# RhushabhVaghela/Custom-NVComp-with-ZSTD

Hardware: AMD Instinct MI355X
Metric: compress GB/s + ratio, 1 GB @ level 3, 64 KB chunks; libzstd round-trip OK (higher is better)
Workload: dtype u8; 1 GPU; C3: 16384 x 64 KiB chunks (1.00 GiB), level 3, independent frames; chunk_bytes=65536, chunks_total=16384, chunks_rank0=16384, level=3, parallelism=dp1 (contiguous chunk shards, RCCL all-gather of sizes inside the step), gathered_frame_bytes=388747049

## Files before the change

custom-nvcomp-with-zstd_amd/csrc/zh_lz.hip:

```cpp
#include "zh_common.h"
#include "zh_hash.h"
#include "zh_litpack.h"

#include <algorithm>
#include <type_traits>
#include <vector>

#if defined(ZH_STAMPS) || defined(ZH_INS_CHECK)
__device__ u32 g_fixups;
extern "C" __global__ void zh_read_fixups(u32 *out) { *out = g_fixups; g_fixups = 0; }
extern "C" u32 zh_fixups_host() {
  u32 *d = nullptr, h = 0;
  if (hipMalloc(&d, 4) != hipSuccess) return ~0u;
  hipLaunchKernelGGL(zh_read_fixups, dim3(1), dim3(1), 0, 0, d);
  (void)hipMemcpy(&h, d, 4, hipMemcpyDeviceToHost);
  (void)hipFree(d);
  return h;
}
#endif
#ifdef ZH_TIMELINE
__device__ unsigned long long g_tl[16 * 8];
extern "C" __global__ void zh_read_timeline(unsigned long long *out) {
  for (u32 i = threadIdx.x; i < 16 * 8; i += blockDim.x) { out[i] = g_tl[i]; g_tl[i] = 0; }
}
extern "C" int zh_timeline_host(unsigned long long *out128) {
  unsigned long long *d = nullptr;
  if (hipMalloc(&d, 16 * 8 * 8) != hipSuccess) return 1;
  hipLaunchKernelGGL(zh_read_timeline, dim3(1), dim3(128), 0, 0, d);
  hipError_t e = hipMemcpy(out128, d, 16 * 8 * 8, hipMemcpyDeviceToHost);
  (void)hipFree(d);
  return e == hipSuccess ? 0 : 1;
}
#define TL_DECL u64 tl_[6] = {0, 0, 0, 0, 0, 0}; u64 tl_prev = __builtin_amdgcn_s_memtime()
#define TL_MARK(ph) do { u64 const _t = __builtin_amdgcn_s_memtime(); tl_[ph] += _t - tl_prev; tl_prev = _t; } while (0)
#define TL_STEP() (tl_[5]++)
#define TL_FLUSH(w, lane) do { if ((lane) == 0) for (u32 _i = 0; _i < 6; _i++) atomicAdd(&g_tl[(w) * 8 + _i], (unsigned long long)tl_[_i]); } while (0)
#else
#define TL_DECL do { } while (0)
#define TL_MARK(ph) do { } while (0)
#define TL_STEP() do { } while (0)
#define TL_FLUSH(w, lane) do { } while (0)
#endif
namespace {

constexpr u32 K1_THREADS = 1024;
constexpr u32 K1_REDO = ~0u;
constexpr u32 NROUND = ZH_WINDOW / 64;
constexpr u32 SEGP = 32;
constexpr u32 NSEG = ZH_WINDOW / SEGP;
constexpr u32 INS_TID = 896;
constexpr u64 ROUND_TAB = 0x6abfff8ull;
constexpr u32 NWW = INS_TID / 64;
constexpr u32 TILES = ZH_WINDOW / ZH_TILE;
constexpr u32 TPL = ZH_TILE / 64;
constexpr u32 NCR = TILES * TPL / 2;
static_assert(NSEG == 64, "one walk lane per segment");
static_assert(INS_TID == 896 && NROUND == 32, "round split: waves 1..13 take 2, 7 x 3, 4 x 2 and 1 rounds");
static_assert((ROUND_TAB & 3) == 0 && (ROUND_TAB >> (2 * (INS_TID / 64))) == 0, "no length rounds on wave 0 or the inserters");
constexpr u32 REC_WAVE = 1;
static_assert(ZH_WINDOW % ZH_TILE == 0 && ZH_TILE % 64 == 0 && TILES * TPL % 2 == 0, "tiles tile windows");

constexpr u32 HL_SIZE = 1u << ZH_HASH_LOG_LONG;
constexpr u32 HS_SIZE = 1u << ZH_HASH_LOG_SHORT;
constexpr u32 T_PAD = 8;
constexpr u32 OFF_IN = 0;
constexpr u32 OFF_TL = OFF_IN + ZH_BLOCK_MAX + 16;
constexpr u32 OFF_TS = OFF_TL + 2 * (HL_SIZE + T_PAD);
constexpr u32 OFF_CI = OFF_TS + 2 * (HS_SIZE + T_PAD);
constexpr u32 CI_WORDS = ZH_WINDOW + 8;
__device__ __forceinline__ u32 cidx(u32 i) { return i; }
constexpr u32 OFF_HM = OFF_CI + 2 * 4 * CI_WORDS;
constexpr u32 LM_BUFS = 3;
constexpr u32 LB_BUFS = 2;
constexpr u32 STEPS_EXTRA = 3;
constexpr u32 OFF_SEGM = OFF_HM + 2 * 8 * NROUND;
__device__ __forceinline__ u32 segm(u32 par) { return par * NSEG; }
constexpr u32 ML_CAP = ((ZH_WINDOW + ZH_MIN_MATCH_SHORT - 1) / ZH_MIN_MATCH_SHORT + 12 + 3) & ~3u;
constexpr u32 OFF_ML = OFF_SEGM + 4 * LM_BUFS * NSEG;
constexpr u32 XQ_CAP = 196;
constexpr u32 OFF_XQ = OFF_ML + 2 * 8 * ML_CAP;
constexpr u32 OFF_MISC = OFF_XQ + 2 * XQ_CAP * NWW;
constexpr u32 OFF_LB = OFF_MISC + 4 * 16;
constexpr u32 LB_WORDS = NSEG + 4;
constexpr u32 K1_LDS = OFF_LB + 4 * LB_WORDS * LB_BUFS;
constexpr u32 ML_LO = 11, ML_LEN = 22, ML_OFF = 29, ML_CUM = 45;
constexpr u32 MISC_WNM = 0;
constexpr u32 MISC_PF = 12;
constexpr u32 MISC_NM = 4;
constexpr u32 MISC_ANY = 13;
constexpr u32 MISC_SCAN = 2;
constexpr u32 MISC_XCH = 8;
constexpr u32 MISC_RESF = 14;
static_assert(K1_LDS <= 163840 - 256, "K1 LDS budget");
static_assert(OFF_TL % 16 == 0 && OFF_CI % 16 == 0 && OFF_HM % 16 == 0 && OFF_MISC % 4 == 0, "alignment");


__device__ __forceinline__ u32 ffbl_raw(u32 x) {
  u32 r;
  __asm__("v_ffbl_b32 %0, %1" : "=v"(r) : "v"(x));
  return r;
}

constexpr u32 K1_DYN = 16;
__device__ __forceinline__ u8 *k1_lds() { return (u8 *)(__attribute__((address_space(3))) u8 *)(uintptr_t)K1_DYN; }

__device__ __forceinline__ void k1_barrier() {
  __builtin_amdgcn_fence(__ATOMIC_RELEASE, "workgroup", "local");
  __builtin_amdgcn_s_barrier();
  __builtin_amdgcn_fence(__ATOMIC_ACQUIRE, "workgroup", "local");
}

__device__ __forceinline__ void ld64u(const u32 *in32, u32 p, u32 &lo, u32 &hi) {
  u32 const w = p >> 2, sh = p & 3;
  u32 const w0 = in32[w], w1 = in32[w + 1], w2 = in32[w + 2];
  lo = __builtin_amdgcn_alignbyte(w1, w0, sh);
  hi = __builtin_amdgcn_alignbyte(w2, w1, sh);
}
// ... 710 lines not shown
    const u32 *const lm = sgm + segm(j % LM_BUFS);
    const u32 *const lb = lbx + (j & 1u) * LB_WORDS;
    if (nr) {
      if constexpr (DW) lit_rounds(in32, lm, lb, lit_out, nlit, wsj, r0, nr, lane);
      else lit_rounds_pos((const u8 *)in32, lm, lb, lit_out, nlit, wsj, r0, nr, lane);
    }
    nlit += (u32)__builtin_amdgcn_readfirstlane(lb[NSEG]);
  }
};
template <class LJ>
__device__ __forceinline__ bool idle_inserter_loop(u32 *misc_, u32 n, u32 wstart, u32 kprobe, u32 e0p, LJ &lj, u32 lane, bool lazy) {
  u32 const nwin = (n - wstart + ZH_WINDOW - 1) / ZH_WINDOW;
  for (u32 k = 0; k < nwin + STEPS_EXTRA; k++) {
    if (probe_dead(misc_, k, kprobe)) return true;
    k1_barrier();
    u32 const wsb = wstart + k * ZH_WINDOW;
    if (probe_dead_tm(k, kprobe, e0p, lazy, min(wsb, n) - (wsb - ZH_WINDOW))) return true;
    lj.step(k, lane);
  }
  return false;
}
template <bool LONG, bool TWO, class LJ>
__device__ __forceinline__ bool inserter_loop(const u32 *in32, u16 *T, u8 *ci8, u32 *misc_, u32 n, u32 lim, u32 lane, u32 *dbg, u32 wstart,
                                              u32 pmin, u32 span_s, u32 span_e, u32 kskip0, u32 kprobe, u32 e0p, LJ &lj, bool lazy) {
  u32 creg[NCR];
  if (span_s < span_e) insert_span<LONG>(in32, T, span_s, span_e, lane);
  insert_window<LONG, true>(in32, T, wstart, lim, lane, creg, NoCheck{}, false, pmin);
  u32 cwe = lookahead<LONG>(in32, T, min(wstart + (u32)ZH_WINDOW, n), lim, lane);
  bool skipc = false;
#ifdef ZH_STAMPS
  u32 st_ins = 0;
#endif
  u32 const nwin = (n - wstart + ZH_WINDOW - 1) / ZH_WINDOW;
  TL_DECL;
  for (u32 k = 0; k < nwin + STEPS_EXTRA; k++) {
    if (probe_dead(misc_, k, kprobe)) return true;
    u32 const wsb = wstart + k * ZH_WINDOW;
    if (k < nwin) {
      for (u32 it = 0; it < (1u << 22) && (u32)__builtin_amdgcn_readfirstlane(__atomic_load_n(&misc_[MISC_PF], __ATOMIC_RELAXED)) < k; it++)
        __builtin_amdgcn_s_sleep(1);
      TL_MARK(3);
      if (skipc) dump_window<LONG, ZH_SKIP_TILES>(ci8 + (k & 1u) * 4 * CI_WORDS, lane, creg, cwe);
      else dump_window<LONG, TILES>(ci8 + (k & 1u) * 4 * CI_WORDS, lane, creg, cwe);
    }
    TL_MARK(4);
    k1_barrier();
    TL_MARK(0);
    TL_STEP();
    if (probe_dead_tm(k, kprobe, e0p, lazy, min(wsb, n) - (wsb - ZH_WINDOW))) return true;
#ifdef ZH_STAMPS
    u64 const ti0 = __builtin_amdgcn_s_memtime();
#endif
    u32 const nx = wsb + ZH_WINDOW;
    skipc = skip_window(misc_, k + 1, kskip0);
    if (k + 1 < nwin) {
      bool resumed = false;
      auto const on_check = [&](bool h) { return resumed = resume_exchange<LONG, TWO>(misc_, k + 1, h, lane); };
      if (nx + ZH_WINDOW <= lim) insert_window<LONG, false>(in32, T, nx, lim, lane, creg, on_check, skipc, 0u);
      else insert_window<LONG, true>(in32, T, nx, lim, lane, creg, on_check, skipc, 0u);
      if (resumed) skipc = false;
      cwe = lookahead<LONG>(in32, T, min(nx + ZH_WINDOW, n), lim, lane);
    }
#ifdef ZH_STAMPS
    st_ins += (u32)(__builtin_amdgcn_s_memtime() - ti0);
#endif
    TL_MARK(1);
    lj.step(k, lane);
    TL_MARK(2);
  }
  TL_FLUSH(LONG ? 14u : 15u, lane);
#ifdef ZH_STAMPS
  if (LONG && lane == 0) dbg[16] = st_ins;
#endif
  (void)dbg;
  return false;
}

}

#ifdef ZH_STAMPS
#define ZH_STAMP(acc)                                           \
  do {                                                          \
    u64 _t = __builtin_amdgcn_s_memtime();                      \
    acc += (u32)(_t - stamp_prev);                              \
    stamp_prev = _t;                                            \
  } while (0)
#else
#define ZH_STAMP(acc) do { } while (0)
#endif

struct Prefetch {
  uint4 v[4];
  bool ok;
};
__device__ __forceinline__ const u8 *staged_region(const ZhBlockDesc &d, u32 &n) {
  u32 const pre = d.pre_n;
  n = pre + d.n;
  const u8 *const g = (pre && d.pre + pre == d.src) ? d.pre : (pre ? nullptr : d.src);
  return (d.n && g && (((uintptr_t)g) & 15) == 0 && (pre & 15) == 0 && (n & 15) == 0) ? g : nullptr;
}
__device__ __forceinline__ void prefetch_block(const ZhBlockDesc *__restrict__ blocks, u32 b, u32 nblocks, u32 tid, Prefetch &pf) {
  pf.ok = false;
  if (b >= nblocks) return;
  ZhBlockDesc const d = blocks[b];
  u32 n;
  const u8 *const g = staged_region(d, n);
  if (!g) return;
  pf.ok = true;
#pragma unroll
  for (u32 k = 0; k < 4; k++) {
    u32 const i = tid + K1_THREADS * k;
    pf.v[k] = i < (n >> 4) ? ((const uint4 *)g)[i] : make_uint4(0, 0, 0, 0);
  }
}

constexpr u64 K1_WAVE_MAP = 0xFEDCBA9876543210ull;
__device__ __forceinline__ bool block_any(bool v, u32 *flag, u32 tid) {
  if (__ballot(v) && (tid & 63) == 0) atomicOr(flag, 1u);
  k1_barrier();
  bool const r = *flag != 0;
  k1_barrier();
  if (tid == 0) *flag = 0;
  k1_barrier();
  return r;
}

__device__ __forceinline__ u32 k1_tid(u32 w) {
  u32 lane;
  __asm__ volatile("v_mbcnt_lo_u32_b32 %0, -1, 0\n\tv_mbcnt_hi_u32_b32 %0, -1, %0" : "=v"(lane));
  return (u32)((K1_WAVE_MAP >> (4 * w)) & 15u) << 6 | lane;
}
// ... 47 lines not shown
#pragma unroll
    for (u32 k = 0; k < 6; k++) w[k] = in32[j0 + k];
#pragma unroll
    for (u32 k = 0; k < 5; k++) v[k] = __builtin_amdgcn_alignbyte(w[k + 1], w[k], sh);
    u32 const lo[4] = {v[0], __builtin_amdgcn_alignbyte(v[1], v[0], 3), __builtin_amdgcn_alignbyte(v[2], v[1], 2), __builtin_amdgcn_alignbyte(v[3], v[2], 1)};
    u32 const hi[4] = {v[1], __builtin_amdgcn_alignbyte(v[2], v[1], 3), __builtin_amdgcn_alignbyte(v[3], v[2], 2), __builtin_amdgcn_alignbyte(v[4], v[3], 1)};
    u32 t[4], e[4];
#pragma unroll
    for (u32 u = 0; u < 4; u++) {
      t[u] = hash_long_sum(lo[u], hi[u]);
      e[u] = *slot(t[u]);
    }
#pragma unroll
    for (u32 u = 0; u < 4; u++) c += (4u * g + u < nm && e[u] - key(t[u]) < p0 + 3u * u) ? 1u : 0u;
  }
  u32 const wsum = lane_value(wave_scan_incl(c), 63);
  if (lane == 0 && wsum) atomicAdd(&misc[MISC_SCAN], wsum);
  k1_barrier();
  u32 const total = (u32)__builtin_amdgcn_readfirstlane(__atomic_load_n(&misc[MISC_SCAN], __ATOMIC_RELAXED));
  return total >= max(span >> ZH_SCAN_SHIFT, (u32)ZH_SCAN_MIN);
}

template <u32 MODE, bool SET>
__device__ __forceinline__ u32 lz_block(const ZhBlockDesc *__restrict__ blocks, ZhWorkspace ws, u32 b, u32 nblocks, u32 *s_take, Prefetch &pf, u32 wv, bool redo) {
  u8 *const smem = k1_lds();
  u8 *in = smem + OFF_IN;
  u32 *in32 = (u32 *)in;
  u16 *TL = (u16 *)(smem + OFF_TL), *TS = (u16 *)(smem + OFF_TS);
  u32 *ci = (u32 *)(smem + OFF_CI);
  u8 *ci8 = smem + OFF_CI;
  u64 *hm = (u64 *)(smem + OFF_HM);
  u32 *misc = (u32 *)(smem + OFF_MISC);

  u32 tid;
  __asm__ volatile("v_mov_b32 %0, %1" : "=v"(tid) : "v"(k1_tid(wv)));
  u32 const lane = tid & 63;
  ZhBlockDesc const d = blocks[b];
  if (tid == 0 && !redo) *s_take = atomicAdd(ws.ctr, 1u);
  if (d.n == 0) {
    k1_barrier();
    u32 const next_b = *s_take;
    prefetch_block(blocks, next_b, nblocks, tid, pf);
    return next_b;
  }
  u32 const pre = d.pre_n;
  u32 const n = pre + d.n;
  u32 *meta = ws.meta(b);
#ifdef ZH_STAMPS
  u64 const rt0 = __builtin_amdgcn_s_memrealtime();
  u64 stamp_prev = __builtin_amdgcn_s_memtime();
  u64 const mt0 = stamp_prev;
  u32 st_stage = 0, st_A = 0, st_X = 0, st_E1 = 0, st_Bmax = 0, st_Imax = 0, st_Bw = 0, st_B = 0, st_J = 0, st_E = 0, st_E2 = 0, st_rounds = 0, st_J1 = 0, st_J2 = 0, st_J3 = 0;
#endif

  const u8 *src = d.src;
  bool same = true;
  u32 nst;
  if (!redo && pf.ok && staged_region(d, nst)) {
    u32 const nv = n >> 4, pv = pre >> 4;
    u32 const f4 = src[0] * 0x01010101u;
#pragma unroll
    for (u32 k = 0; k < 4; k++) {
      u32 const i = tid + K1_THREADS * k;
      uint4 const v = pf.v[k];
      if (i < nv) {
// ... 26 lines not shown
  }
  if (tid < 16) in[n + tid] = 0;
  const u16 *dtab = ws.dtab;
  u32 dtab_P = ws.dtab_P;
  if constexpr (SET) {
    if ((d.flags & ZH_F_DICT) && (d.flags & ZH_F_FIRST)) {
      const ZhDictSetEntry *const e = ws.set + ws.item_ent[d.item];
      dtab_P = e->dtab_P;
      dtab = dtab_P ? e->dtab : nullptr;
    }
  }
  bool const use_dt = dtab && (d.flags & ZH_F_DICT) && (d.flags & ZH_F_FIRST) && pre >= 2 * ZH_DTAB_MARGIN && d.n >= 16 &&
                      dtab_P >= pre;
  bool const par_hist = !use_dt && pre >= 2 * ZH_TILE && d.n >= 16;
  u32 const pmin = (use_dt || par_hist) ? pre & ~(ZH_TILE - 1) : 0u;
  u32 const wstart = (use_dt || par_hist) ? (pre & ~(ZH_WINDOW - 1)) : 0u;
  u32 const span_s = use_dt ? pre - ZH_DTAB_MARGIN : 0u, span_e = use_dt ? pmin : 0u;
  u32 const kskip0 = pre / ZH_WINDOW + 3 - wstart / ZH_WINDOW;
  u32 const lim = n > ZH_HASH_READ ? n - ZH_HASH_READ : 0;
  u32 const a0 = pre / ZH_WINDOW, nwl = (lim + ZH_WINDOW - 1) / ZH_WINDOW;
  u32 const e0p = pre - a0 * ZH_WINDOW;
  u32 const kprobe0 = a0 + ZH_PROBE_WINDOWS + 1 <= nwl && e0p <= ZH_PROBE_MAX_E0 ? a0 + ZH_PROBE_WINDOWS + 1 - wstart / ZH_WINDOW : ~0u;
  u32 next_b = 0;
  if (use_dt) {
    u32 const delta = dtab_P - pre;
    const u32 *dt32 = (const u32 *)dtab;
    auto clip = [&](u32 e) { return e > delta ? e - delta : 0u; };
    for (u32 i = tid; i < (HL_SIZE + HS_SIZE) / 2; i += K1_THREADS) {
      u32 const w = dt32[i];
      u32 const v = clip(w & 0xFFFFu) | (clip(w >> 16) << 16);
      u32 const j = i < HL_SIZE / 2 ? i : i + T_PAD / 2;
      ((u32 *)TL)[j] = v;
    }
    if (tid < T_PAD) ((u16 *)TL)[tid < T_PAD / 2 ? HL_SIZE + tid : HL_SIZE + T_PAD + HS_SIZE + (tid - T_PAD / 2)] = 0;
  } else {
    for (u32 i = tid; i < (HL_SIZE + HS_SIZE + 2 * T_PAD) / 2; i += K1_THREADS) ((u32 *)TL)[i] = 0;
  }
  if (tid == 0) {
    misc[MISC_PF] = 0;
#pragma unroll
    for (u32 i = 0; i < 4; i++) misc[MISC_XCH + i] = 0;
  }
  if (!redo) {
    bool const rle = !block_any(!same, &misc[MISC_ANY], tid) && d.n >= 2;
    next_b = *s_take;
    prefetch_block(blocks, next_b, nblocks, tid, pf);
    if (rle) {
      if (tid == 0) {
        u32 one;
        __asm__ volatile("v_mov_b32 %0, 1" : "=v"(one));
        meta[0] = one - 1u; meta[1] = one - 1u; meta[2] = one;
      }
      return next_b;
    }
  } else {
    next_b = *s_take;
    k1_barrier();
  }
  if (par_hist) {
    for (u32 round = 0;; round++) {
      bool ch = false;
      for (u32 p = tid; p < pmin; p += K1_THREADS) {
        u32 lo, hi;
        ld64u(in32, p, lo, hi);
        u32 const hl = hash_of<true>(lo, hi), hs = hash_of<false>(lo, hi);
        u16 const v = (u16)(p + 1);
        if (round == 0) {
          TL[hl] = v;
          TS[hs] = v;
        } else {
          if (TL[hl] < v) { TL[hl] = v; ch = true; }
          if (TS[hs] < v) { TS[hs] = v; ch = true; }
        }
      }
      if (round == 0) k1_barrier();
      else if (!block_any(ch, &misc[MISC_ANY], tid)) break;
    }
  }

  ZH_STAMP(st_stage);
  u32 const kprobe = redo ? ~0u : kprobe0;
  bool dead = false;
  if (tid >= INS_TID) {
    __builtin_amdgcn_s_setprio(2);
    bool const lw = tid < INS_TID + 64;
    LitJob<two_tables<MODE>()> lj{in32, (u32 *)(smem + OFF_SEGM), (u32 *)(smem + OFF_LB), ws.lits(b), wstart, n, pre,
              two_tables<MODE>() && !lw ? LIT_ROUNDS / 2 : 0u, two_tables<MODE>() ? LIT_ROUNDS / 2 : (lw ? LIT_ROUNDS : 0u), 0u};
    if (tid >= INS_TID + 64)
      dead = inserter_loop<false, two_tables<MODE>()>(in32, TS, ci8, misc, n, lim, lane, ws.dbg(b), wstart, pmin, span_s, span_e, kskip0, kprobe, e0p, lj,
                                                      MODE != 2);
    else if (two_tables<MODE>())
      dead = inserter_loop<true, true>(in32, TL, ci8, misc, n, lim, lane, ws.dbg(b), wstart, pmin, span_s, span_e, kskip0, kprobe, e0p, lj, MODE != 2);
    else
      dead = idle_inserter_loop(misc, n, wstart, kprobe, e0p, lj, lane, MODE != 2);
    __builtin_amdgcn_s_setprio(0);
    if (!dead) return next_b;
  } else {
  u64 *const seq_out = ws.seq(b);
  u32 nseq_tot = 0, nlit_tot = 0, e_in = pre;
  u32 const tid_ = tid;
  u32 const wave = tid >> 6;
  u32 r_lo = 0;
  for (u32 w = 0; w < wave; w++) r_lo += rounds_of_mode<MODE>(w);
  u32 const r_hi = r_lo + rounds_of_mode<MODE>(wave);
  u32 *const ci0 = ci;
  u32 *const sgm = (u32 *)(smem + OFF_SEGM);
  u32 *const lbx = (u32 *)(smem + OFF_LB);
  u16 *const xq = (u16 *)(smem + OFF_XQ) + XQ_CAP * wave;
  u32 const nwin = (n - wstart + ZH_WINDOW - 1) / ZH_WINDOW;
  u64 *const mlist = (u64 *)(smem + OFF_ML);
  u32 nwalk_tot = 0;
  TL_DECL;
  u32 m3 = 0;
  bool skp_prev = false;
  for (u32 k = 0; k < nwin + STEPS_EXTRA; k++, m3 = m3 + 1 == LM_BUFS ? 0u : m3 + 1) {
    if (probe_dead(misc, k, kprobe)) {
      dead = true;
      break;
    }
    u32 const wsb = wstart + k * ZH_WINDOW;
    u32 const we = min(wsb + ZH_WINDOW, n);
    u32 const kb = k & 1u;
    bool const have = k < nwin && we > pre;
    u32 const wsp = wsb - ZH_WINDOW, wep = min(wsp + ZH_WINDOW, n);
    bool const prev = k >= 1 && k <= nwin && wep > pre;
    u32 const wsq = wsb - 2 * ZH_WINDOW;
    bool const prev2 = k >= 2 && k - 2 < nwin && min(wsq + ZH_WINDOW, n) > pre;
    u32 tid;
    __asm__ volatile("v_mov_b32 %0, %1" : "=v"(tid) : "v"(tid_));
    u32 const lane = tid & 63;
    u32 *const ciK = ci0 + kb * CI_WORDS, *const ciP = ci0 + (kb ^ 1u) * CI_WORDS;
    u64 *const tmK = hm + kb * NROUND, *const tmP = hm + (kb ^ 1u) * NROUND;
    static_assert(LM_BUFS == 3 && LB_BUFS == 2, "literal buffer rotation");
    u32 *const lmP = sgm + segm(m3 == 0 ? 2u : m3 - 1u);
    u32 *const lmQ = sgm + segm(m3 == 0 ? 1u : m3 == 1 ? 2u : 0u);
    u32 *const lbxq = lbx + kb * LB_WORDS;
    u64 *const mlP = mlist + (kb ^ 1u) * ML_CAP, *const mlQ = mlist + kb * ML_CAP;
    k1_barrier();
    TL_MARK(0);
    TL_STEP();
    if (probe_dead_tm(k, kprobe, e0p, MODE != 2, wep - wsp)) {
      dead = true;
      break;
    }
    ZH_STAMP(st_A);
    constexpr u32 RS = 2 * ZH_SKIP_TILES;
    static_assert(RS < NWW && (RS & 1) == 0, "miss-skip rounds");
    bool const skipk = have && skip_window_eff(misc, k, kskip0);
    if (skipk && wave != 0) {
      if constexpr (MODE == 2) {
        if (wave <= RS / L1_S) span_lengths_l1(in32, ciK, tmK, xq, wave - 1, wave, wsb, n, lane);
      } else {
        if (wave <= RS) span_lengths<MODE, 1>(in32, ciK, tmK, xq, wave - 1, wave, wsb, we, n, lim, lane, wave == RS, 0u);
      }
      for (u32 r = RS + wave - 1; r < NROUND; r += NWW - 1) {
        ciK[cidx(64 * r + lane)] = 0;
        if (lane == 0) tmK[r] = 0;
      }
      ZH_STAMP(st_B);
    } else if (MODE == 2 && have && wave != 0) {
      if (r_lo < r_hi) span_lengths_l1(in32, ciK, tmK, xq, r_lo, r_hi, wsb, n, lane);
      ZH_STAMP(st_B);
    } else if (have && wave != 0) {
      u32 la1 = 0;
      if (wave == NWW - 1) {
// ... 104 lines not shown
        if (v) seq_out[nseq_tot + j] = (u64)cum | ((u64)len << 17) | ((u64)e << 24) | ((u64)off << 36);
        if (e) {
          for (u32 g = (ms - e) / SEGP; g <= (ms - 1) / SEGP; g++) {
            u32 const a = max(ms - e, SEGP * g) - SEGP * g, bnd = min(ms - SEGP * g, SEGP);
            atomicAnd(&lmQ[g], ~bit_range32(a, bnd));
          }
        }
      }
      u32 const lc = (u32)__popc(lmQ[lane]), lincl = wave_scan_incl(lc);
      lbxq[lane] = lincl - lc;
      if (lane == 63) lbxq[NSEG] = lincl;
      nlit_tot += lane_value(lincl, 63);
      nseq_tot += nm;
    }
    if (wave != 0) TL_MARK(2);
    TL_MARK(3);
    ZH_STAMP(st_X);
    ZH_STAMP(st_E);
    TL_MARK(4);
    skp_prev = skipk;
  }
  TL_FLUSH(wave, lane);
  if (!dead) {
    if (tid_ == 64u * REC_WAVE) { meta[0] = nseq_tot; meta[1] = nlit_tot; meta[2] = 0; }
#ifdef ZH_STAMPS
    if (tid == 0) {
      u32 *dbg = ws.dbg(b);
      dbg[23] = (u32)rt0; dbg[24] = (u32)__builtin_amdgcn_s_memrealtime();
      dbg[25] = __builtin_amdgcn_s_getreg((31 << 11) | 4);
      dbg[26] = __builtin_amdgcn_s_getreg((31 << 11) | 20);
      dbg[27] = (u32)(__builtin_amdgcn_s_memtime() - mt0);
      dbg[40] = st_Bmax; dbg[41] = st_Imax; dbg[55] = st_J1; dbg[56] = st_J2; dbg[57] = st_J3;
      dbg[0] = st_stage; dbg[1] = st_A; dbg[2] = st_B; dbg[3] = st_J; dbg[4] = st_E; dbg[5] = st_rounds; dbg[20] = st_E2; dbg[21] = st_X; dbg[22] = st_E1;
    }
    if ((tid & 63) == 0 && tid < INS_TID) {
      u32 const w = tid >> 6;
      ws.dbg(b)[w < 12 ? 28 + w : 53 + (w - 12)] = st_B;
    }
#endif
    return next_b;
  }
  }
  u32 *const hw = (u32 *)(smem + OFF_CI);
  if (repeat_scan(in32, (u32 *)TL, hw, misc, pre, n, tid)) return K1_REDO;
  ZH_STAMP(st_E1);
  u32 const wave = tid >> 6;
// ... 25 lines not shown
    u32 w[5];
#pragma unroll
    for (u32 k = 0; k < 5; k++) w[k] = src32[4 * i + k];
    uint4 v;
    v.x = __builtin_amdgcn_alignbyte(w[1], w[0], sh);
    v.y = __builtin_amdgcn_alignbyte(w[2], w[1], sh);
    v.z = __builtin_amdgcn_alignbyte(w[3], w[2], sh);
    v.w = __builtin_amdgcn_alignbyte(w[4], w[3], sh);
    ((uint4 *)lit_out)[i] = v;
  }
  if (tid == 0) { meta[0] = 0; meta[1] = d.n; meta[2] = 0; }
  return next_b;
}

template <u32 MODE, bool SET = false>
__device__ __forceinline__ void lz_blocks(const ZhBlockDesc *__restrict__ blocks, u32 nblocks, ZhWorkspace ws) {
  extern __shared__ __attribute__((aligned(16))) u8 smem_dyn[];
  u8 *const smem = k1_lds();
  if (threadIdx.x == 0 && (u32)(uintptr_t)smem_dyn != K1_DYN) __builtin_trap();
  __shared__ u32 s_take;
  if (threadIdx.x == 0) {
    s_take = atomicAdd(ws.ctr, 1u);
    ((u32 *)(smem + OFF_MISC))[MISC_ANY] = 0;
  }
  k1_barrier();
  u32 b = s_take;
  Prefetch pf;
  u32 const wv = (u32)__builtin_amdgcn_readfirstlane(threadIdx.x >> 6);
  prefetch_block(blocks, b, nblocks, k1_tid(wv), pf);
  bool redo = false;
  while (b < nblocks) {
    u32 const r = (u32)__builtin_amdgcn_readfirstlane(lz_block<MODE, SET>(blocks, ws, b, nblocks, &s_take, pf, wv, redo));
    k1_barrier();
    redo = r == K1_REDO;
    b = redo ? b : r;
  }
}
extern "C" __global__ __launch_bounds__(K1_THREADS) void zh_lz_kernel(const ZhBlockDesc *__restrict__ blocks, u32 nblocks, ZhWorkspace ws) {
  lz_blocks<0>(blocks, nblocks, ws);
}
extern "C" __global__ __launch_bounds__(K1_THREADS) void zh_lz_short_kernel(const ZhBlockDesc *__restrict__ blocks, u32 nblocks, ZhWorkspace ws) {
  lz_blocks<1>(blocks, nblocks, ws);
}
extern "C" __global__ __launch_bounds__(K1_THREADS) void zh_lz_greedy_kernel(const ZhBlockDesc *__restrict__ blocks, u32 nblocks, ZhWorkspace ws) {
  lz_blocks<2>(blocks, nblocks, ws);
}
extern "C" __global__ __launch_bounds__(K1_THREADS) void zh_lz_set_kernel(const ZhBlockDesc *__restrict__ blocks, u32 nblocks, ZhWorkspace ws) {
  lz_blocks<0, true>(blocks, nblocks, ws);
}
extern "C" __global__ __launch_bounds__(K1_THREADS) void zh_lz_short_set_kernel(const ZhBlockDesc *__restrict__ blocks, u32 nblocks, ZhWorkspace ws) {
  lz_blocks<1, true>(blocks, nblocks, ws);
}
extern "C" __global__ __launch_bounds__(K1_THREADS) void zh_lz_greedy_set_kernel(const ZhBlockDesc *__restrict__ blocks, u32 nblocks, ZhWorkspace ws) {
  lz_blocks<2, true>(blocks, nblocks, ws);
}
template <u32 MODE>
// ... 35 lines not shown

namespace zh {
hipError_t lz_init() {
  for (const void *f : {(const void *)zh_lz_kernel, (const void *)zh_lz_short_kernel, (const void *)zh_lz_greedy_kernel,
                        (const void *)zh_lz_ranged_kernel, (const void *)zh_lz_short_ranged_kernel, (const void *)zh_lz_greedy_ranged_kernel,
                        (const void *)zh_lz_set_kernel, (const void *)zh_lz_short_set_kernel, (const void *)zh_lz_greedy_set_kernel}) {
    hipError_t const e = hipFuncSetAttribute(f, hipFuncAttributeMaxDynamicSharedMemorySize, (int)K1_LDS);
    if (e != hipSuccess) return e;
  }
  return hipSuccess;
}
u32 lz_dict_tables_P(size_t cn) {
  u32 const P = (u32)std::min(cn, (size_t)65535);
  return P < 2 * ZH_DTAB_MARGIN ? 0u : P;
}
hipError_t lz_dict_tables_batch(const ZhDictBuildJob *d_jobs, u32 count, u32 *tmp32, hipStream_t stream) {
  if (!count) return hipSuccess;
  hipError_t e = hipMemsetAsync(tmp32, 0, (size_t)count * 4 * (HL_SIZE + HS_SIZE), stream);
  if (e != hipSuccess) return e;
  hipLaunchKernelGGL(zh_dict_hash_batch_kernel, dim3((65535 - ZH_DTAB_MARGIN + 255) / 256, count), dim3(256), 0, stream, d_jobs, tmp32);
  hipLaunchKernelGGL(zh_dict_pack_batch_kernel, dim3((HL_SIZE + HS_SIZE + 255) / 256, count), dim3(256), 0, stream, d_jobs, (const u32 *)tmp32);
  return hipGetLastError();
}
void lz_launch(const ZhBlockDesc *d_descs, u32 nblocks, ZhWorkspace ws, u32 mode, hipStream_t stream) {
  int dev = 0, cus = 0;
  if (stream) (void)hipStreamGetDevice(stream, &dev);
  else (void)hipGetDevice(&dev);
  if (hipDeviceGetAttribute(&cus, hipDeviceAttributeMultiprocessorCount, dev) != hipSuccess || cus <= 0) cus = 256;
  u32 const grid = std::min(nblocks, (u32)cus);
  auto *const k = ws.set ? (mode == 2 ? zh_lz_greedy_set_kernel : mode == 1 ? zh_lz_short_set_kernel : zh_lz_set_kernel)
                         : (mode == 2 ? zh_lz_greedy_kernel : mode == 1 ? zh_lz_short_kernel : zh_lz_kernel);
  hipLaunchKernelGGL(k, dim3(grid), dim3(K1_THREADS), K1_LDS, stream, d_descs, nblocks, ws);
}
void lz_launch_ranged(const ZhBlockDesc *d_descs, u32 nblocks, ZhWorkspace ws, ZhClassRanges *d_ranges, hipStream_t stream) {
  int dev = 0, cus = 0;
  if (stream) (void)hipStreamGetDevice(stream, &dev);
  else (void)hipGetDevice(&dev);
  if (hipDeviceGetAttribute(&cus, hipDeviceAttributeMultiprocessorCount, dev) != hipSuccess || cus <= 0) cus = 256;
  u32 const grid = std::min(nblocks, (u32)cus);
  for (auto *const k : {zh_lz_greedy_ranged_kernel, zh_lz_short_ranged_kernel, zh_lz_ranged_kernel})
    hipLaunchKernelGGL(k, dim3(grid), dim3(K1_THREADS), K1_LDS, stream, d_descs, d_ranges, ws);
}
}

extern "C" void zh_test_lz_sizes(u32 *seq_cap, u32 *lit_bytes) { *seq_cap = ZH_SEQ_CAP; *lit_bytes = ZH_LIT_BYTES; }
extern "C" int zh_test_lz(const u8 *d_in, u32 nitems, u32 stride, const u32 *h_sizes, int mode, u64 *h_recs, u8 *h_lits, u32 *h_meta) {
  if (!nitems) return 0;
  std::vector<ZhBlockDesc> descs(nitems);
  for (u32 i = 0; i < nitems; i++) {
    if (h_sizes[i] > ZH_BLOCK_MAX) return 2;
    ZhBlockDesc d{};
    d.src = d_in + (size_t)i * stride;
    d.n = h_sizes[i];
    d.frame_size = h_sizes[i];
    d.item = i;
    d.flags = ZH_F_FIRST | ZH_F_LAST | ZH_F_DIRECT;
    descs[i] = d;
  }
  ZhBlockDesc *dd = nullptr;
  u8 *base = nullptr;
  u32 *ctr = nullptr;
  int rc = 0;
  if (zh::lz_init() != hipSuccess || hipMalloc(&dd, sizeof(ZhBlockDesc) * nitems) != hipSuccess ||
      hipMalloc(&base, (size_t)ZH_WS_BLOCK_BYTES * nitems) != hipSuccess || hipMalloc(&ctr, 4) != hipSuccess) {
    rc = 1;
  } else {
    (void)hipMemcpy(dd, descs.data(), sizeof(ZhBlockDesc) * nitems, hipMemcpyHostToDevice);
    (void)hipMemset(ctr, 0, 4);
    ZhWorkspace ws{base, ctr, nullptr, 0u};
    zh::lz_launch(dd, nitems, ws, (u32)mode, nullptr);
    if (hipDeviceSynchronize() != hipSuccess) rc = 1;
    for (u32 i = 0; i < nitems && !rc; i++) {
      u8 *const b = base + (size_t)i * ZH_WS_BLOCK_BYTES;
      (void)hipMemcpy(h_recs + (size_t)i * ZH_SEQ_CAP, b, ZH_SEQ_BYTES, hipMemcpyDeviceToHost);
      (void)hipMemcpy(h_lits + (size_t)i * ZH_LIT_BYTES, b + ZH_SEQ_BYTES, ZH_LIT_BYTES, hipMemcpyDeviceToHost);
      (void)hipMemcpy(h_meta + 4 * i, b + ZH_SEQ_BYTES + ZH_LIT_BYTES, 16, hipMemcpyDeviceToHost);
    }
  }
  (void)hipFree(dd);
  (void)hipFree(base);
  (void)hipFree(ctr);
  return rc;
}
```

Before: 92.95 GB/s.

## Pre-insert next block's first window into hash tables during current block's drain

During the drain steps at the end of a block, the inserter waves load the next block's first window into a new LDS shadow buffer, clear their hash table, insert that window and dump its candidates. The next block then skips its own table clearing and first-window insertion, which overlaps block-boundary startup with the previous block's tail. The table zeroing also becomes 16-byte vector stores. In exchange this adds LDS use, restructures the inserter loop into body and tail variants, and adds cross-block state that must stay consistent on redo paths.

```diff
diff --git a/custom-nvcomp-with-zstd_amd/csrc/zh_k1_boundary.h b/custom-nvcomp-with-zstd_amd/csrc/zh_k1_boundary.h
--- /dev/null
+++ b/custom-nvcomp-with-zstd_amd/csrc/zh_k1_boundary.h
@@ -0,0 +1,65 @@
+#pragma once
+#include "zh_block_plan.h"
+
+#if defined(__HIPCC__)
+#define ZH_K1B_HD __host__ __device__ inline
+#else
+#define ZH_K1B_HD inline
+#endif
+
+namespace zh_k1 {
+
+constexpr u32 K1_THREADS = 1024;
+constexpr u32 NROUND = ZH_WINDOW / 64;
+constexpr u32 SEGP = 32;
+constexpr u32 NSEG = ZH_WINDOW / SEGP;
+constexpr u32 INS_TID = 896;
+constexpr u32 NWW = INS_TID / 64;
+
+constexpr u32 HL_SIZE = 1u << ZH_HASH_LOG_LONG;
+constexpr u32 HS_SIZE = 1u << ZH_HASH_LOG_SHORT;
+constexpr u32 T_PAD = 8;
+constexpr u32 OFF_IN = 0;
+constexpr u32 OFF_TL = OFF_IN + ZH_BLOCK_MAX + 16;
+constexpr u32 OFF_TS = OFF_TL + 2 * (HL_SIZE + T_PAD);
+constexpr u32 OFF_CI = OFF_TS + 2 * (HS_SIZE + T_PAD);
+constexpr u32 CI_WORDS = ZH_WINDOW + 8;
+constexpr u32 OFF_HM = OFF_CI + 2 * 4 * CI_WORDS;
+constexpr u32 LM_BUFS = 3;
+constexpr u32 LB_BUFS = 2;
+constexpr u32 OFF_SEGM = OFF_HM + 2 * 8 * NROUND;
+constexpr u32 ML_CAP = ((ZH_WINDOW + ZH_MIN_MATCH_SHORT - 1) / ZH_MIN_MATCH_SHORT + 12 + 3) & ~3u;
+constexpr u32 OFF_ML = OFF_SEGM + 4 * LM_BUFS * NSEG;
+constexpr u32 XQ_CAP = 196;
+constexpr u32 XQ_WAVES = NWW - 1;
+constexpr u32 OFF_XQ = OFF_ML + 2 * 8 * ML_CAP;
+constexpr u32 OFF_MISC = OFF_XQ + 2 * XQ_CAP * XQ_WAVES;
+constexpr u32 MISC_WORDS = 16;
+constexpr u32 OFF_LB = OFF_MISC + 4 * MISC_WORDS;
+constexpr u32 LB_WORDS = NSEG + 4;
+constexpr u32 SHADOW_BYTES = ZH_WINDOW + 16;
+constexpr u32 OFF_SHADOW = (OFF_LB + 4 * LB_WORDS * LB_BUFS + 15u) & ~15u;
+constexpr u32 K1_LDS = OFF_SHADOW + SHADOW_BYTES;
+constexpr u32 K1_LDS_BUDGET = 163840 - 256;
+static_assert(K1_LDS <= K1_LDS_BUDGET, "K1 LDS budget");
+static_assert(OFF_TL % 16 == 0 && OFF_TS % 16 == 0 && OFF_CI % 16 == 0 && OFF_HM % 16 == 0 && OFF_MISC % 4 == 0 && OFF_SHADOW % 16 == 0,
+              "alignment");
+
+ZH_K1B_HD const u8 *zh_k1_staged_region(const ZhBlockDesc &d, u32 &n) {
+  u32 const pre = d.pre_n;
+  n = pre + d.n;
+  const u8 *const g = (pre && d.pre + pre == d.src) ? d.pre : (pre ? nullptr : d.src);
+  return (d.n && g && (((uintptr_t)g) & 15) == 0 && (pre & 15) == 0 && (n & 15) == 0) ? g : nullptr;
+}
+
+constexpr u32 ZH_K1_PRE_MIN = ZH_WINDOW + 16;
+static_assert(ZH_K1_PRE_MIN >= SHADOW_BYTES && ZH_K1_PRE_MIN > ZH_WINDOW + 1 + ZH_HASH_READ, "the lookahead positions are below lim");
+
+ZH_K1B_HD u32 zh_k1_windows(u32 n, u32 wstart) { return (n - wstart + ZH_WINDOW - 1) / ZH_WINDOW; }
+
+ZH_K1B_HD bool zh_k1_preinsert(bool next_ok, u32 next_pre_n, u32 next_n, bool redo, u32 nwin) {
+  return next_ok && next_pre_n == 0 && next_n >= ZH_K1_PRE_MIN && !redo && nwin >= 3;
+}
+ZH_K1B_HD u32 zh_k1_predump_step(u32 nwin) { return nwin + (nwin & 1u) + 1u; }
+
+}
diff --git a/custom-nvcomp-with-zstd_amd/csrc/zh_lz.hip b/custom-nvcomp-with-zstd_amd/csrc/zh_lz.hip
--- a/custom-nvcomp-with-zstd_amd/csrc/zh_lz.hip
+++ b/custom-nvcomp-with-zstd_amd/csrc/zh_lz.hip
@@ -1,5 +1,6 @@
 #include "zh_common.h"
 #include "zh_hash.h"
+#include "zh_k1_boundary.h"
 #include "zh_litpack.h"
 
 #include <algorithm>
@@ -19,15 +20,16 @@
 }
 #endif
 #ifdef ZH_TIMELINE
-__device__ unsigned long long g_tl[16 * 8];
+constexpr unsigned ZH_TL_WORDS = 16 * 8 + 8;
+__device__ unsigned long long g_tl[ZH_TL_WORDS];
 extern "C" __global__ void zh_read_timeline(unsigned long long *out) {
-  for (u32 i = threadIdx.x; i < 16 * 8; i += blockDim.x) { out[i] = g_tl[i]; g_tl[i] = 0; }
-}
-extern "C" int zh_timeline_host(unsigned long long *out128) {
+  for (u32 i = threadIdx.x; i < ZH_TL_WORDS; i += blockDim.x) { out[i] = g_tl[i]; g_tl[i] = 0; }
+}
+extern "C" int zh_timeline_host(unsigned long long *out136) {
   unsigned long long *d = nullptr;
-  if (hipMalloc(&d, 16 * 8 * 8) != hipSuccess) return 1;
+  if (hipMalloc(&d, ZH_TL_WORDS * 8) != hipSuccess) return 1;
   hipLaunchKernelGGL(zh_read_timeline, dim3(1), dim3(128), 0, 0, d);
-  hipError_t e = hipMemcpy(out128, d, 16 * 8 * 8, hipMemcpyDeviceToHost);
+  hipError_t e = hipMemcpy(out136, d, ZH_TL_WORDS * 8, hipMemcpyDeviceToHost);
   (void)hipFree(d);
   return e == hipSuccess ? 0 : 1;
 }
@@ -35,7 +37,17 @@
 #define TL_MARK(ph) do { u64 const _t = __builtin_amdgcn_s_memtime(); tl_[ph] += _t - tl_prev; tl_prev = _t; } while (0)
 #define TL_STEP() (tl_[5]++)
 #define TL_FLUSH(w, lane) do { if ((lane) == 0) for (u32 _i = 0; _i < 6; _i++) atomicAdd(&g_tl[(w) * 8 + _i], (unsigned long long)tl_[_i]); } while (0)
+#define TB_PARAM , u64 &tb_prev
+#define TB_ARG , tb_prev
+#define TB_MARK(i, t) do { u64 const _t = __builtin_amdgcn_s_memtime(); if (tb_prev && (t) == 0) atomicAdd(&g_tl[128 + (i)], (unsigned long long)(_t - tb_prev)); tb_prev = _t; } while (0)
+#define TB_COUNT(t) do { if (tb_prev && (t) == 0) atomicAdd(&g_tl[133], 1ull); } while (0)
+#define TB_RESET() (tb_prev = 0)
 #else
+#define TB_PARAM
+#define TB_ARG
+#define TB_MARK(i, t) do { } while (0)
+#define TB_COUNT(t) do { } while (0)
+#define TB_RESET() do { } while (0)
 #define TL_DECL do { } while (0)
 #define TL_MARK(ph) do { } while (0)
 #define TL_STEP() do { } while (0)
@@ -43,14 +55,9 @@
 #endif
 namespace {
 
-constexpr u32 K1_THREADS = 1024;
+using namespace zh_k1;
 constexpr u32 K1_REDO = ~0u;
-constexpr u32 NROUND = ZH_WINDOW / 64;
-constexpr u32 SEGP = 32;
-constexpr u32 NSEG = ZH_WINDOW / SEGP;
-constexpr u32 INS_TID = 896;
 constexpr u64 ROUND_TAB = 0x6abfff8ull;
-constexpr u32 NWW = INS_TID / 64;
 constexpr u32 TILES = ZH_WINDOW / ZH_TILE;
 constexpr u32 TPL = ZH_TILE / 64;
 constexpr u32 NCR = TILES * TPL / 2;
@@ -60,29 +67,9 @@
 constexpr u32 REC_WAVE = 1;
 static_assert(ZH_WINDOW % ZH_TILE == 0 && ZH_TILE % 64 == 0 && TILES * TPL % 2 == 0, "tiles tile windows");
 
-constexpr u32 HL_SIZE = 1u << ZH_HASH_LOG_LONG;
-constexpr u32 HS_SIZE = 1u << ZH_HASH_LOG_SHORT;
-constexpr u32 T_PAD = 8;
-constexpr u32 OFF_IN = 0;
-constexpr u32 OFF_TL = OFF_IN + ZH_BLOCK_MAX + 16;
-constexpr u32 OFF_TS = OFF_TL + 2 * (HL_SIZE + T_PAD);
-constexpr u32 OFF_CI = OFF_TS + 2 * (HS_SIZE + T_PAD);
-constexpr u32 CI_WORDS = ZH_WINDOW + 8;
 __device__ __forceinline__ u32 cidx(u32 i) { return i; }
-constexpr u32 OFF_HM = OFF_CI + 2 * 4 * CI_WORDS;
-constexpr u32 LM_BUFS = 3;
-constexpr u32 LB_BUFS = 2;
 constexpr u32 STEPS_EXTRA = 3;
-constexpr u32 OFF_SEGM = OFF_HM + 2 * 8 * NROUND;
 __device__ __forceinline__ u32 segm(u32 par) { return par * NSEG; }
-constexpr u32 ML_CAP = ((ZH_WINDOW + ZH_MIN_MATCH_SHORT - 1) / ZH_MIN_MATCH_SHORT + 12 + 3) & ~3u;
-constexpr u32 OFF_ML = OFF_SEGM + 4 * LM_BUFS * NSEG;
-constexpr u32 XQ_CAP = 196;
-constexpr u32 OFF_XQ = OFF_ML + 2 * 8 * ML_CAP;
-constexpr u32 OFF_MISC = OFF_XQ + 2 * XQ_CAP * NWW;
-constexpr u32 OFF_LB = OFF_MISC + 4 * 16;
-constexpr u32 LB_WORDS = NSEG + 4;
-constexpr u32 K1_LDS = OFF_LB + 4 * LB_WORDS * LB_BUFS;
 constexpr u32 ML_LO = 11, ML_LEN = 22, ML_OFF = 29, ML_CUM = 45;
 constexpr u32 MISC_WNM = 0;
 constexpr u32 MISC_PF = 12;
@@ -91,8 +78,9 @@
 constexpr u32 MISC_SCAN = 2;
 constexpr u32 MISC_XCH = 8;
 constexpr u32 MISC_RESF = 14;
+constexpr u32 MISC_PRE = 3;
 static_assert(K1_LDS <= 163840 - 256, "K1 LDS budget");
-static_assert(OFF_TL % 16 == 0 && OFF_CI % 16 == 0 && OFF_HM % 16 == 0 && OFF_MISC % 4 == 0, "alignment");
+static_assert(STEPS_EXTRA == 3 && MISC_PRE < MISC_WORDS && MISC_RESF + 1 < MISC_WORDS, "the drain has a step for the next block's dump");
 
 
 __device__ __forceinline__ u32 ffbl_raw(u32 x) {
@@ -849,26 +837,49 @@
 }
 template <bool LONG, bool TWO, class LJ>
 __device__ __forceinline__ bool inserter_loop(const u32 *in32, u16 *T, u8 *ci8, u32 *misc_, u32 n, u32 lim, u32 lane, u32 *dbg, u32 wstart,
-                                              u32 pmin, u32 span_s, u32 span_e, u32 kskip0, u32 kprobe, u32 e0p, LJ &lj, bool lazy) {
+                                              u32 pmin, u32 span_s, u32 span_e, u32 kskip0, u32 kprobe, u32 e0p, LJ &lj, bool lazy,
+                                              bool pre_done, u32 nxn, u32 nxb, const ZhBlockDesc *__restrict__ blocks) {
   u32 creg[NCR];
-  if (span_s < span_e) insert_span<LONG>(in32, T, span_s, span_e, lane);
-  insert_window<LONG, true>(in32, T, wstart, lim, lane, creg, NoCheck{}, false, pmin);
-  u32 cwe = lookahead<LONG>(in32, T, min(wstart + (u32)ZH_WINDOW, n), lim, lane);
+  u32 cwe = 0;
+  if (!pre_done) {
+    if (span_s < span_e) insert_span<LONG>(in32, T, span_s, span_e, lane);
+    insert_window<LONG, true>(in32, T, wstart, lim, lane, creg, NoCheck{}, false, pmin);
+    cwe = lookahead<LONG>(in32, T, min(wstart + (u32)ZH_WINDOW, n), lim, lane);
+  }
   bool skipc = false;
 #ifdef ZH_STAMPS
   u32 st_ins = 0;
 #endif
-  u32 const nwin = (n - wstart + ZH_WINDOW - 1) / ZH_WINDOW;
+  u32 const nwin = zh_k1_windows(n, wstart);
+  u32 const kdump = nxn ? zh_k1_predump_step(nwin) : ~0u;
   TL_DECL;
-  for (u32 k = 0; k < nwin + STEPS_EXTRA; k++) {
+  auto step = [&](u32 k, auto tail_c) __attribute__((always_inline)) -> bool {
+    constexpr bool TAIL = decltype(tail_c)::value;
     if (probe_dead(misc_, k, kprobe)) return true;
     u32 const wsb = wstart + k * ZH_WINDOW;
-    if (k < nwin) {
+    constexpr u32 SHV = SHADOW_BYTES / 16 - 1;
+    static_assert(SHV == 128, "two rows of 64 vectors and one more");
+    bool const fill = TAIL && nxn != 0 && k + 1 == nwin;
+    uint4 sv0 = make_uint4(0, 0, 0, 0), sv1 = sv0, sv2 = sv0;
+    if (fill) {
+      const uint4 *const g = (const uint4 *)blocks[nxb].src;
+      if (!TWO || LONG) { sv0 = g[lane]; sv2 = g[SHV]; }
+      if (!TWO || !LONG) sv1 = g[64 + lane];
+    }
+    if (TAIL && k == kdump) {
+      TL_MARK(3);
+      dump_window<LONG, TILES>(ci8, lane, creg, cwe);
+    } else if ((!TAIL || k < nwin) && !(pre_done && k == 0)) {
       for (u32 it = 0; it < (1u << 22) && (u32)__builtin_amdgcn_readfirstlane(__atomic_load_n(&misc_[MISC_PF], __ATOMIC_RELAXED)) < k; it++)
         __builtin_amdgcn_s_sleep(1);
       TL_MARK(3);
       if (skipc) dump_window<LONG, ZH_SKIP_TILES>(ci8 + (k & 1u) * 4 * CI_WORDS, lane, creg, cwe);
       else dump_window<LONG, TILES>(ci8 + (k & 1u) * 4 * CI_WORDS, lane, creg, cwe);
+    }
+    if (fill) {
+      uint4 *const sh = (uint4 *)(k1_lds() + OFF_SHADOW);
+      if (!TWO || LONG) { sh[lane] = sv0; if (lane == 0) sh[SHV] = sv2; }
+      if (!TWO || !LONG) sh[64 + lane] = sv1;
     }
     TL_MARK(4);
     k1_barrier();
@@ -878,9 +889,9 @@
 #ifdef ZH_STAMPS
     u64 const ti0 = __builtin_amdgcn_s_memtime();
 #endif
-    u32 const nx = wsb + ZH_WINDOW;
-    skipc = skip_window(misc_, k + 1, kskip0);
-    if (k + 1 < nwin) {
+    if constexpr (!TAIL) {
+      u32 const nx = wsb + ZH_WINDOW;
+      skipc = skip_window(misc_, k + 1, kskip0);
       bool resumed = false;
       auto const on_check = [&](bool h) { return resumed = resume_exchange<LONG, TWO>(misc_, k + 1, h, lane); };
       if (nx + ZH_WINDOW <= lim) insert_window<LONG, false>(in32, T, nx, lim, lane, creg, on_check, skipc, 0u);
@@ -894,7 +905,25 @@
     TL_MARK(1);
     lj.step(k, lane);
     TL_MARK(2);
-  }
+    if (TAIL && nxn != 0 && k + 1 == nwin) {
+      u32 zero;
+      __asm__ volatile("v_mov_b32 %0, 0" : "=v"(zero));
+      constexpr u32 TV = 2 * ((LONG ? HL_SIZE : HS_SIZE) + T_PAD) / 16;
+      static_assert(2 * (HL_SIZE + T_PAD) % 16 == 0 && 2 * (HS_SIZE + T_PAD) % 16 == 0, "a table is whole 16-B vectors");
+      for (u32 i = lane; i < TV; i += 64) ((uint4 *)T)[i] = make_uint4(zero, zero, zero, zero);
+      const u32 *const sh32 = (const u32 *)(k1_lds() + OFF_SHADOW);
+      u32 const nlim = nxn - (u32)ZH_HASH_READ;
+      insert_window<LONG, true>(sh32, T, 0u, nlim, lane, creg, NoCheck{}, false, 0u);
+      cwe = lookahead<LONG>(sh32, T, min((u32)ZH_WINDOW, nxn), nlim, lane);
+      if (!LONG && lane == 0) misc_[MISC_PRE] = nxb + 1u;
+      TL_MARK(1);
+    }
+    return false;
+  };
+  for (u32 k = 0; k + 1 < nwin; k++)
+    if (step(k, std::false_type{})) return true;
+  for (u32 k = nwin - 1; k < nwin + STEPS_EXTRA; k++)
+    if (step(k, std::true_type{})) return true;
   TL_FLUSH(LONG ? 14u : 15u, lane);
 #ifdef ZH_STAMPS
   if (LONG && lane == 0) dbg[16] = st_ins;
@@ -919,21 +948,20 @@
 struct Prefetch {
   uint4 v[4];
   bool ok;
+  u32 bn, bpre;
 };
-__device__ __forceinline__ const u8 *staged_region(const ZhBlockDesc &d, u32 &n) {
-  u32 const pre = d.pre_n;
-  n = pre + d.n;
-  const u8 *const g = (pre && d.pre + pre == d.src) ? d.pre : (pre ? nullptr : d.src);
-  return (d.n && g && (((uintptr_t)g) & 15) == 0 && (pre & 15) == 0 && (n & 15) == 0) ? g : nullptr;
-}
+__device__ __forceinline__ const u8 *staged_region(const ZhBlockDesc &d, u32 &n) { return zh_k1_staged_region(d, n); }
 __device__ __forceinline__ void prefetch_block(const ZhBlockDesc *__restrict__ blocks, u32 b, u32 nblocks, u32 tid, Prefetch &pf) {
   pf.ok = false;
+  pf.bn = pf.bpre = 0;
   if (b >= nblocks) return;
   ZhBlockDesc const d = blocks[b];
   u32 n;
   const u8 *const g = staged_region(d, n);
   if (!g) return;
   pf.ok = true;
+  pf.bn = d.n;
+  pf.bpre = d.pre_n;
 #pragma unroll
   for (u32 k = 0; k < 4; k++) {
     u32 const i = tid + K1_THREADS * k;
@@ -1027,7 +1055,7 @@
 }
 
 template <u32 MODE, bool SET>
-__device__ __forceinline__ u32 lz_block(const ZhBlockDesc *__restrict__ blocks, ZhWorkspace ws, u32 b, u32 nblocks, u32 *s_take, Prefetch &pf, u32 wv, bool redo) {
+__device__ __forceinline__ u32 lz_block(const ZhBlockDesc *__restrict__ blocks, ZhWorkspace ws, u32 b, u32 nblocks, u32 *s_take, Prefetch &pf, u32 wv, bool redo TB_PARAM) {
   u8 *const smem = k1_lds();
   u8 *in = smem + OFF_IN;
   u32 *in32 = (u32 *)in;
@@ -1046,6 +1074,7 @@
     k1_barrier();
     u32 const next_b = *s_take;
     prefetch_block(blocks, next_b, nblocks, tid, pf);
+    TB_RESET();
     return next_b;
   }
   u32 const pre = d.pre_n;
@@ -1118,6 +1147,8 @@
   u32 const e0p = pre - a0 * ZH_WINDOW;
   u32 const kprobe0 = a0 + ZH_PROBE_WINDOWS + 1 <= nwl && e0p <= ZH_PROBE_MAX_E0 ? a0 + ZH_PROBE_WINDOWS + 1 - wstart / ZH_WINDOW : ~0u;
   u32 next_b = 0;
+  bool const pre_done = !redo && (u32)__builtin_amdgcn_readfirstlane(misc[MISC_PRE]) == b + 1u;
+  u32 nxn = 0;
   if (use_dt) {
     u32 const delta = dtab_P - pre;
     const u32 *dt32 = (const u32 *)dtab;
@@ -1129,8 +1160,11 @@
       ((u32 *)TL)[j] = v;
     }
     if (tid < T_PAD) ((u16 *)TL)[tid < T_PAD / 2 ? HL_SIZE + tid : HL_SIZE + T_PAD + HS_SIZE + (tid - T_PAD / 2)] = 0;
-  } else {
-    for (u32 i = tid; i < (HL_SIZE + HS_SIZE + 2 * T_PAD) / 2; i += K1_THREADS) ((u32 *)TL)[i] = 0;
+  } else if (!pre_done) {
+    u32 zero;
+    __asm__ volatile("v_mov_b32 %0, 0" : "=v"(zero));
+    static_assert((HL_SIZE + HS_SIZE + 2 * T_PAD) % 8 == 0, "the tables are whole 16-B vectors");
+    for (u32 i = tid; i < (HL_SIZE + HS_SIZE + 2 * T_PAD) / 8; i += K1_THREADS) ((uint4 *)TL)[i] = make_uint4(zero, zero, zero, zero);
   }
   if (tid == 0) {
     misc[MISC_PF] = 0;
@@ -1141,12 +1175,16 @@
     bool const rle = !block_any(!same, &misc[MISC_ANY], tid) && d.n >= 2;
     next_b = *s_take;
     prefetch_block(blocks, next_b, nblocks, tid, pf);
+    u32 const nn = (u32)__builtin_amdgcn_readfirstlane(pf.bn), npre = (u32)__builtin_amdgcn_readfirstlane(pf.bpre);
+    bool const nok = (u32)__builtin_amdgcn_readfirstlane(pf.ok ? 1u : 0u) != 0;
+    nxn = zh_k1_preinsert(nok, npre, nn, redo, zh_k1_windows(n, wstart)) ? nn : 0u;
     if (rle) {
       if (tid == 0) {
         u32 one;
         __asm__ volatile("v_mov_b32 %0, 1" : "=v"(one));
         meta[0] = one - 1u; meta[1] = one - 1u; meta[2] = one;
       }
+      TB_RESET();
       return next_b;
     }
   } else {
@@ -1175,6 +1213,7 @@
   }
 
   ZH_STAMP(st_stage);
+  TB_MARK(2, tid);
   u32 const kprobe = redo ? ~0u : kprobe0;
   bool dead = false;
   if (tid >= INS_TID) {
@@ -1182,11 +1221,13 @@
     bool const lw = tid < INS_TID + 64;
     LitJob<two_tables<MODE>()> lj{in32, (u32 *)(smem + OFF_SEGM), (u32 *)(smem + OFF_LB), ws.lits(b), wstart, n, pre,
               two_tables<MODE>() && !lw ? LIT_ROUNDS / 2 : 0u, two_tables<MODE>() ? LIT_ROUNDS / 2 : (lw ? LIT_ROUNDS : 0u), 0u};
+    u32 const nxb = (u32)__builtin_amdgcn_readfirstlane(next_b);
     if (tid >= INS_TID + 64)
       dead = inserter_loop<false, two_tables<MODE>()>(in32, TS, ci8, misc, n, lim, lane, ws.dbg(b), wstart, pmin, span_s, span_e, kskip0, kprobe, e0p, lj,
-                                                      MODE != 2);
+                                                      MODE != 2, pre_done, nxn, nxb, blocks);
     else if (two_tables<MODE>())
-      dead = inserter_loop<true, true>(in32, TL, ci8, misc, n, lim, lane, ws.dbg(b), wstart, pmin, span_s, span_e, kskip0, kprobe, e0p, lj, MODE != 2);
+      dead = inserter_loop<true, true>(in32, TL, ci8, misc, n, lim, lane, ws.dbg(b), wstart, pmin, span_s, span_e, kskip0, kprobe, e0p, lj, MODE != 2,
+                                       pre_done, nxn, nxb, blocks);
     else
       dead = idle_inserter_loop(misc, n, wstart, kprobe, e0p, lj, lane, MODE != 2);
     __builtin_amdgcn_s_setprio(0);
@@ -1202,8 +1243,8 @@
   u32 *const ci0 = ci;
   u32 *const sgm = (u32 *)(smem + OFF_SEGM);
   u32 *const lbx = (u32 *)(smem + OFF_LB);
-  u16 *const xq = (u16 *)(smem + OFF_XQ) + XQ_CAP * wave;
-  u32 const nwin = (n - wstart + ZH_WINDOW - 1) / ZH_WINDOW;
+  u16 *const xq = (u16 *)(smem + OFF_XQ) + XQ_CAP * (wave ? wave - 1u : 0u);
+  u32 const nwin = zh_k1_windows(n, wstart);
   u64 *const mlist = (u64 *)(smem + OFF_ML);
   u32 nwalk_tot = 0;
   TL_DECL;
@@ -1212,6 +1253,7 @@
   for (u32 k = 0; k < nwin + STEPS_EXTRA; k++, m3 = m3 + 1 == LM_BUFS ? 0u : m3 + 1) {
     if (probe_dead(misc, k, kprobe)) {
       dead = true;
+      TB_RESET();
       break;
     }
     u32 const wsb = wstart + k * ZH_WINDOW;
@@ -1235,8 +1277,11 @@
     k1_barrier();
     TL_MARK(0);
     TL_STEP();
+    if (k == 0) TB_MARK(3, tid_);
+    if (k == nwin) TB_MARK(4, tid_);
     if (probe_dead_tm(k, kprobe, e0p, MODE != 2, wep - wsp)) {
       dead = true;
+      TB_RESET();
       break;
     }
     ZH_STAMP(st_A);
@@ -1387,6 +1432,8 @@
   }
   TL_FLUSH(wave, lane);
   if (!dead) {
+    TB_COUNT(tid_);
+    TB_MARK(0, tid_);
     if (tid_ == 64u * REC_WAVE) { meta[0] = nseq_tot; meta[1] = nlit_tot; meta[2] = 0; }
 #ifdef ZH_STAMPS
     if (tid == 0) {
@@ -1458,6 +1505,7 @@
   if (threadIdx.x == 0) {
     s_take = atomicAdd(ws.ctr, 1u);
     ((u32 *)(smem + OFF_MISC))[MISC_ANY] = 0;
+    ((u32 *)(smem + OFF_MISC))[MISC_PRE] = 0;
   }
   k1_barrier();
   u32 b = s_take;
@@ -1465,9 +1513,13 @@
   u32 const wv = (u32)__builtin_amdgcn_readfirstlane(threadIdx.x >> 6);
   prefetch_block(blocks, b, nblocks, k1_tid(wv), pf);
   bool redo = false;
+#ifdef ZH_TIMELINE
+  u64 tb_prev = 0;
+#endif
   while (b < nblocks) {
-    u32 const r = (u32)__builtin_amdgcn_readfirstlane(lz_block<MODE, SET>(blocks, ws, b, nblocks, &s_take, pf, wv, redo));
+    u32 const r = (u32)__builtin_amdgcn_readfirstlane(lz_block<MODE, SET>(blocks, ws, b, nblocks, &s_take, pf, wv, redo TB_ARG));
     k1_barrier();
+    TB_MARK(1, threadIdx.x);
     redo = r == K1_REDO;
     b = redo ? b : r;
   }
@@ -1549,15 +1601,18 @@
   hipLaunchKernelGGL(zh_dict_pack_batch_kernel, dim3((HL_SIZE + HS_SIZE + 255) / 256, count), dim3(256), 0, stream, d_jobs, (const u32 *)tmp32);
   return hipGetLastError();
 }
-void lz_launch(const ZhBlockDesc *d_descs, u32 nblocks, ZhWorkspace ws, u32 mode, hipStream_t stream) {
+static void lz_launch_grid(const ZhBlockDesc *d_descs, u32 nblocks, ZhWorkspace ws, u32 mode, hipStream_t stream, u32 max_grid) {
   int dev = 0, cus = 0;
   if (stream) (void)hipStreamGetDevice(stream, &dev);
   else (void)hipGetDevice(&dev);
   if (hipDeviceGetAttribute(&cus, hipDeviceAttributeMultiprocessorCount, dev) != hipSuccess || cus <= 0) cus = 256;
-  u32 const grid = std::min(nblocks, (u32)cus);
+  u32 const grid = std::min(std::min(nblocks, (u32)cus), max_grid);
   auto *const k = ws.set ? (mode == 2 ? zh_lz_greedy_set_kernel : mode == 1 ? zh_lz_short_set_kernel : zh_lz_set_kernel)
                          : (mode == 2 ? zh_lz_greedy_kernel : mode == 1 ? zh_lz_short_kernel : zh_lz_kernel);
   hipLaunchKernelGGL(k, dim3(grid), dim3(K1_THREADS), K1_LDS, stream, d_descs, nblocks, ws);
+}
+void lz_launch(const ZhBlockDesc *d_descs, u32 nblocks, ZhWorkspace ws, u32 mode, hipStream_t stream) {
+  lz_launch_grid(d_descs, nblocks, ws, mode, stream, ~0u);
 }
 void lz_launch_ranged(const ZhBlockDesc *d_descs, u32 nblocks, ZhWorkspace ws, ZhClassRanges *d_ranges, hipStream_t stream) {
   int dev = 0, cus = 0;
@@ -1571,13 +1626,15 @@
 }
 
 extern "C" void zh_test_lz_sizes(u32 *seq_cap, u32 *lit_bytes) { *seq_cap = ZH_SEQ_CAP; *lit_bytes = ZH_LIT_BYTES; }
-extern "C" int zh_test_lz(const u8 *d_in, u32 nitems, u32 stride, const u32 *h_sizes, int mode, u64 *h_recs, u8 *h_lits, u32 *h_meta) {
+extern "C" int zh_test_lz_grid(const u8 *d_in, u32 nitems, const u64 *h_offs, const u32 *h_sizes, int mode, u32 grid, u64 *h_recs, u8 *h_lits,
+                               u32 *h_meta) {
   if (!nitems) return 0;
+  if (!grid) return 2;
   std::vector<ZhBlockDesc> descs(nitems);
   for (u32 i = 0; i < nitems; i++) {
     if (h_sizes[i] > ZH_BLOCK_MAX) return 2;
     ZhBlockDesc d{};
-    d.src = d_in + (size_t)i * stride;
+    d.src = d_in + h_offs[i];
     d.n = h_sizes[i];
     d.frame_size = h_sizes[i];
     d.item = i;
@@ -1595,7 +1652,7 @@
     (void)hipMemcpy(dd, descs.data(), sizeof(ZhBlockDesc) * nitems, hipMemcpyHostToDevice);
     (void)hipMemset(ctr, 0, 4);
     ZhWorkspace ws{base, ctr, nullptr, 0u};
-    zh::lz_launch(dd, nitems, ws, (u32)mode, nullptr);
+    zh::lz_launch_grid(dd, nitems, ws, (u32)mode, nullptr, grid);
     if (hipDeviceSynchronize() != hipSuccess) rc = 1;
     for (u32 i = 0; i < nitems && !rc; i++) {
       u8 *const b = base + (size_t)i * ZH_WS_BLOCK_BYTES;
@@ -1609,3 +1666,8 @@
   (void)hipFree(ctr);
   return rc;
 }
+extern "C" int zh_test_lz(const u8 *d_in, u32 nitems, u32 stride, const u32 *h_sizes, int mode, u64 *h_recs, u8 *h_lits, u32 *h_meta) {
+  std::vector<u64> offs(nitems);
+  for (u32 i = 0; i < nitems; i++) offs[i] = (u64)i * stride;
+  return zh_test_lz_grid(d_in, nitems, offs.data(), h_sizes, mode, ~0u, h_recs, h_lits, h_meta);
+}
```

Measured after the change: 93.67 GB/s (median of 6 runs). About the same (+0.8%).
